# martinsbruveris/tensorflow-image-models

Measured on AMD Instinct MI355X. Metric: images/sec (fwd, bf16), higher is better.
Workload: dtype bf16; 1 GPU; resnet50 @224 fwd; per_gpu_batch=256, global_batch=256, parallelism=dp1, exchange=none, ranks=1, launcher=in-process, launch=hipGraph replay, 2 parallel branches of 128 images, branches=2

## Files before the change

### tensorflow-image-models_amd/csrc/gemm_chain_kernel.h

```cpp
#pragma once
#include "gemm_stream_kernel.h"

namespace tfimm_gemm {

struct ChainArgs {
  const bf16_t* x;
  const bf16_t* w1;
  const float* b1;
  const bf16_t* w2;
  const float* b2;
  const bf16_t* residual;
  const bf16_t* ds_x;
  const uint4* ds_w;
  bf16_t* out;
  int M, N2;
  int B, H, W;
  int ldw1, ldw2, ldr, ldc;
  int act1, act2;
  unsigned x_bytes, w1_bytes, w2_bytes, out_bytes, res_bytes, ds_bytes;
  int n_tiles;
  int dbg;
};

typedef void (*gemm_chain_fn)(const ChainArgs);

struct ChainGeom {
  static constexpr int BM = 128, NW = 4, C1 = 64, BN2 = 64;
  static constexpr int STRIP_ROWS = 256;
  static constexpr int STRIP_BYTES = STRIP_ROWS * 128;
  static constexpr int STAGE = 64 * 128;
#ifndef TFIMM_CHAIN_NST
#define TFIMM_CHAIN_NST 2
#endif
#ifndef TFIMM_CHAIN_WTN
#define TFIMM_CHAIN_WTN 64
#endif
  static constexpr int NST = TFIMM_CHAIN_NST;
  static constexpr int WTN = TFIMM_CHAIN_WTN;
  static constexpr int EPI_WAVE = 32 * WTN * 4;
  static constexpr int LDS_BYTES = STRIP_BYTES + NST * STAGE + NW * EPI_WAVE;
  static_assert(LDS_BYTES <= 80 * 1024, "two workgroups must fit one CU's 160 KiB of LDS");
};

template <int N>
__device__ __forceinline__ void chain_wait_vm() {
  asm volatile("s_waitcnt vmcnt(%0)" ::"n"(N) : "memory");
}

template <int I>
struct ChainIdx {
  static constexpr int value = I;
};

template <int NS2, int ACT = -1, bool DS = false>
__global__ void __launch_bounds__(256, 2) gemm_chain_kernel(const ChainArgs p) {
  using G = ChainGeom;
  constexpr int BM = G::BM, NW = G::NW, STAGE = G::STAGE, BN2 = G::BN2, NST = G::NST;
  constexpr int TN1 = 2;
  constexpr int STRIP_INSTR = G::STRIP_ROWS / 8 / NW;
  constexpr int B1_INSTR = 64 / 8 / NW;
  constexpr int B2_INSTR = BN2 / 8 / NW;
  constexpr int KS2 = 4;
  constexpr int TN2 = BN2 / 32;
  constexpr int NK1 = 9;
  typedef __attribute__((ext_vector_type(4))) unsigned int u32x4;

  extern __shared__ __attribute__((aligned(16))) char smem[];
  char* const sRing = smem + G::STRIP_BYTES;
  float* const sEpi = reinterpret_cast<float*>(smem + G::STRIP_BYTES + NST * STAGE);

  const int tid = threadIdx.x;
  const int lane = tid & 63;
  const int wave = __builtin_amdgcn_readfirstlane(tid >> 6);
  const int frow = lane & 31, fhi = lane >> 5;

  int t_first, t_hi, t_step;
  {
    const int nb = gridDim.x, bid = blockIdx.x;
    const int xcd = bid & 7, j = bid >> 3;
    const int q = p.n_tiles >> 3, r = p.n_tiles & 7;
    const int t_lo = xcd * q + (xcd < r ? xcd : r);
    t_hi = t_lo + q + (xcd < r ? 1 : 0);
    t_step = nb >> 3;
    t_first = t_lo + j;
  }
  if (t_first >= t_hi) return;

  const __amdgpu_buffer_rsrc_t rsrc_x = make_rsrc(p.x, p.x_bytes);
  const __amdgpu_buffer_rsrc_t rsrc_w1 = make_rsrc(p.w1, p.w1_bytes);
  const __amdgpu_buffer_rsrc_t rsrc_w2 = make_rsrc(p.w2, p.w2_bytes);
  const __amdgpu_buffer_rsrc_t rsrc_o = make_rsrc(p.out, p.out_bytes);
  const __amdgpu_buffer_rsrc_t rsrc_r = DS ? make_rsrc(p.ds_x, p.ds_bytes) : make_rsrc(p.residual, p.res_bytes);

  static_assert(NS2 >= 2, "the counted waits below are derived for at least two GEMM-2 steps");
  constexpr int LOOK = NST - 1;
  const int lrow = lane >> 3, lpc = lane & 7;

  unsigned b1_off[B1_INSTR], b2_off[B2_INSTR];
  int strip_chunk[STRIP_INSTR];
#pragma unroll
  for (int j = 0; j < B1_INSTR; ++j) {
    const int r = (wave * B1_INSTR + j) * 8 + lrow;
    b1_off[j] = (unsigned)(((size_t)r * p.ldw1 + (lpc ^ ((r >> 1) & 7)) * 8) * 2);
  }
#pragma unroll
  for (int j = 0; j < B2_INSTR; ++j) {
    const int r = (wave * B2_INSTR + j) * 8 + lrow;
    b2_off[j] = (unsigned)(((size_t)r * p.ldw2 + (lpc ^ ((r >> 1) & 7)) * 8) * 2);
  }
#pragma unroll
  for (int j = 0; j < STRIP_INSTR; ++j) {
    const int r = (wave * STRIP_INSTR + j) * 8 + lrow;
    strip_chunk[j] = (lpc ^ ((r >> 1) & 7)) * 16;
  }
  const int halo = p.W + 1;
  const int n_pix = p.B * p.H * p.W;
  auto issue_strip = [&](int tile, bool valid) __attribute__((always_inline)) {
    const int s0 = tile * BM - halo;
#pragma unroll
    for (int j = 0; j < STRIP_INSTR; ++j) {
      const int r = (wave * STRIP_INSTR + j) * 8 + lrow;
      const int s = s0 + r;
      const bool ok = valid && s >= 0 && s < n_pix;
      const unsigned off = ok ? (unsigned)s * 128u + (unsigned)strip_chunk[j] : kOobOffset;
      __builtin_amdgcn_raw_ptr_buffer_load_lds(rsrc_x, (lds_ptr_t)(smem + (wave * STRIP_INSTR + j) * 1024), 16, (int)off, 0, 0, 0);
    }
  };
  int iss_stage = 0;
  auto issue_step = [&](auto sc, int tile) __attribute__((always_inline)) {
    constexpr int S = decltype(sc)::value;
    constexpr int SL = S >= NK1 + NS2 ? S - NK1 - NS2 : S;
    const bool valid = S >= NK1 + NS2 ? (tile + t_step < t_hi) : true;
    char* const sa = sRing + iss_stage * STAGE;
    if constexpr (SL < NK1) {
#pragma unroll
      for (int j = 0; j < B1_INSTR; ++j) {
        const unsigned off = valid ? b1_off[j] : kOobOffset;
        __builtin_amdgcn_raw_ptr_buffer_load_lds(rsrc_w1, (lds_ptr_t)(sa + (wave * B1_INSTR + j) * 1024), 16, (int)off, SL * 128, 0, 0);
      }
    } else {
      const int soff = (int)((size_t)(SL - NK1) * BN2 * p.ldw2 * 2);
#pragma unroll
      for (int j = 0; j < B2_INSTR; ++j)
        __builtin_amdgcn_raw_ptr_buffer_load_lds(rsrc_w2, (lds_ptr_t)(sa + (wave * B2_INSTR + j) * 1024), 16, (int)b2_off[j], soff, 0, 0);
    }
    iss_stage = iss_stage == NST - 1 ? 0 : iss_stage + 1;
  };

  constexpr int WTN = G::WTN, LPR = WTN / 8, RPI = 64 / LPR, ITS = 32 / RPI;
  constexpr int PASSES = BN2 / WTN;
  constexpr int BPP = WTN / 32;
  constexpr int STORES = PASSES * ITS;
  constexpr int DS_X = DS ? 4 : 0;
  constexpr int DS_W = DS ? 8 : 0;
  constexpr int EPI_LOADS = (DS ? 0 : PASSES * ITS) + PASSES * 2;
  auto epi_slot = [](int row, int slot) -> int { return WTN == 64 ? (slot ^ (row & 15)) : (slot ^ ((row >> 1) & 7)); };
  const ActParams act1p = make_act(ACT >= 0 ? ACT : p.act1), act2p = make_act(ACT >= 0 ? ACT : p.act2);
  const int e_row = lane / LPR, e_c8 = lane % LPR;
  const bool has_res = !DS && p.residual != nullptr;
  float* const sEw = sEpi + wave * (G::EPI_WAVE / 4);

  struct Ops {
    static constexpr int all(int r) {
      if (DS && r == NK1 - 2) return B1_INSTR + TN1 * 4;
      if (r < NK1 - 1) return B1_INSTR;
      if (r == NK1 - 1) return EPI_LOADS + DS_X + B1_INSTR;
      const int u = r - NK1;
      return (u < NS2 - 1 ? EPI_LOADS : 0) + DS_W + B2_INSTR + (u == 0 ? STRIP_INSTR : 0) + STORES;
    }
    static constexpr int behind_dma(int r) {
      if (r < NK1) return 0;
      return (r - NK1 == 0 ? STRIP_INSTR : 0) + STORES;
    }
    static constexpr int wait_for(int r) {
      constexpr int T = NK1 + NS2;
      int n = behind_dma((r + T - LOOK) % T);
      for (int i = 1; i < LOOK; ++i) n += all((r + T - i) % T);
      return n;
    }
  };
  static_assert(B1_INSTR == B2_INSTR, "every weight step is two pieces per wave");
  static_assert(Ops::wait_for(NK1 + NS2 - 1) < 64, "vmcnt is a 6-bit counter");

  f32x4 bias1[TN1][4];
  auto load_bias1 = [&]() __attribute__((always_inline)) {
#pragma unroll
    for (int j = 0; j < TN1; ++j)
#pragma unroll
      for (int q = 0; q < 4; ++q) {
        const float4 b4 = *reinterpret_cast<const float4*>(p.b1 + j * 32 + q * 8 + fhi * 4);
        bias1[j][q] = f32x4{b4.x, b4.y, b4.z, b4.w};
      }
  };
  if constexpr (!DS) {
    load_bias1();
    asm volatile("s_waitcnt vmcnt(0)" : "+v"(bias1[0][0]), "+v"(bias1[0][3]), "+v"(bias1[TN1 - 1][0]), "+v"(bias1[TN1 - 1][3])::"memory");
  }

  if (TFIMM_PROBE(p.dbg) & 8) {
    const int n = ((blockIdx.x >> 3) & 7) * (TFIMM_PROBE(p.dbg) >> 8);
    for (int i = 0; i < n; ++i) asm volatile("s_sleep 8");
  }
  issue_strip(t_first, true);
  issue_step(ChainIdx<0>{}, t_first);
  if constexpr (LOOK > 1) issue_step(ChainIdx<1>{}, t_first);
  if constexpr (LOOK > 2) issue_step(ChainIdx<2>{}, t_first);
  static_assert(LOOK >= 1 && LOOK <= 3, "prologue written for up to three steps of lookahead");
  int cur = 0;
  bool first = true;
  auto rotate = [&]() __attribute__((always_inline)) { cur = cur == NST - 1 ? 0 : cur + 1; };

  for (int tile = t_first; tile < t_hi; tile += t_step) {
    const int m0 = tile * BM;

    unsigned vmask;
    {
      const int m = m0 + wave * 32 + frow;
      const int hw = p.H * p.W;
      const int rem = m % hw;
      const int oy = rem / p.W, ox = rem - oy * p.W;
      const unsigned vy = (oy > 0 ? 1u : 0u) | 2u | (oy + 1 < p.H ? 4u : 0u);
      const unsigned vx = (ox > 0 ? 1u : 0u) | 2u | (ox + 1 < p.W ? 4u : 0u);
      vmask = 0;
#pragma unroll
      for (int ky = 0; ky < 3; ++ky)
        if ((vy >> ky) & 1) vmask |= vx << (3 * ky);
      if (m >= p.M) vmask = 0;
    }

    f32x16 acc1[TN1];
#pragma unroll
    for (int j = 0; j < TN1; ++j)
#pragma unroll
      for (int e = 0; e < 16; ++e) acc1[j][e] = 0.f;
    uint4 rres[2][PASSES][ITS];
    u32x4 dsx[4];
    float4 braw[2][PASSES][2];
    const int e_m = m0 + wave * 32 + e_row;
    const int em = e_m < p.M ? e_m : p.M;
    const unsigned ldc2 = (unsigned)p.ldc * 2u, ldr2 = (unsigned)p.ldr * 2u;
    auto load_epi = [&](auto uc) __attribute__((always_inline)) {
      constexpr int u = decltype(uc)::value;
      const unsigned res_off0 = (unsigned)(((size_t)em * p.ldr + u * BN2 + e_c8 * 8) * 2);
#pragma unroll
      for (int g = 0; g < PASSES; ++g) {
        if constexpr (!DS) {
#pragma unroll
        for (int it = 0; it < ITS; ++it) {
          const unsigned off = res_off0 + (unsigned)(it * RPI) * ldr2 + (unsigned)(g * WTN * 2);
          rres[u & 1][g][it] = __builtin_bit_cast(uint4, __builtin_amdgcn_raw_buffer_load_b128(rsrc_r, (int)((TFIMM_PROBE(p.dbg) & 4) ? kOobOffset : off), 0, 0));
        }
        }
        braw[u & 1][g][0] = *reinterpret_cast<const float4*>(p.b2 + u * BN2 + g * WTN + e_c8 * 8);
        braw[u & 1][g][1] = *reinterpret_cast<const float4*>(p.b2 + u * BN2 + g * WTN + e_c8 * 8 + 4);
      }
    };
    auto tap_step = [&](auto kc) __attribute__((always_inline)) {
      constexpr int k = decltype(kc)::value;
      if constexpr (k < LOOK) { if (first) chain_wait_vm<(LOOK - 1) * B1_INSTR>(); else chain_wait_vm<Ops::wait_for(k)>(); }
      else chain_wait_vm<Ops::wait_for(k)>();
      tfimm_lds_reuse_barrier();
      if constexpr (DS && k == NK1 - 2) { load_bias1(); __builtin_amdgcn_sched_barrier(0); }
      if constexpr (k == NK1 - 1) {
        load_epi(ChainIdx<0>{});
        if constexpr (DS) {
          const unsigned xo = (unsigned)(m0 + wave * 32 + frow) * 128u + (unsigned)fhi * 16u;
#pragma unroll
          for (int t = 0; t < 4; ++t) dsx[t] = __builtin_amdgcn_raw_buffer_load_b128(rsrc_r, (int)(xo + t * 32), 0, 0);
        }
        __builtin_amdgcn_sched_barrier(0);
      }
      issue_step(ChainIdx<k + LOOK>{}, tile);
      if constexpr (k == NK1 - 1) __builtin_amdgcn_sched_barrier(0);
      constexpr int ky = k / 3, kx = k % 3;
      const bool ok = (vmask >> k) & 1;
      const uint4* sB = reinterpret_cast<const uint4*>(sRing + cur * STAGE);
      const int arow = wave * 32 + frow + ky * p.W + kx;
      u32x4 ua[4];
      {
        unsigned ra[4];
#pragma unroll
        for (int ks = 0; ks < 4; ++ks) ra[ks] = (unsigned)(size_t)(lds_ptr_t)(smem + lds_slot(arow, ks * 2 + fhi) * 16);
        asm volatile("ds_read_b128 %0, %4\n\tds_read_b128 %1, %5\n\tds_read_b128 %2, %6\n\tds_read_b128 %3, %7\n\t"
                     "s_waitcnt lgkmcnt(0)"
                     : "=&v"(ua[0]), "=&v"(ua[1]), "=&v"(ua[2]), "=&v"(ua[3])
                     : "v"(ra[0]), "v"(ra[1]), "v"(ra[2]), "v"(ra[3]) : "memory");
      }
#pragma unroll
      for (int ks = 0; ks < 4; ++ks) {
        const uint4 um = sel4(ok, __builtin_bit_cast(uint4, ua[ks]));
        const bf16x8 fa = __builtin_bit_cast(bf16x8, um);
        bf16x8 fb[TN1];
#pragma unroll
        for (int j = 0; j < TN1; ++j) fb[j] = __builtin_bit_cast(bf16x8, sB[lds_slot(j * 32 + frow, ks * 2 + fhi)]);
#pragma unroll
        for (int j = 0; j < TN1; ++j)
          if (!(TFIMM_PROBE(p.dbg) & 2)) acc1[j] = __builtin_amdgcn_mfma_f32_32x32x16_bf16(fb[j], fa, acc1[j], 0, 0, 0);
      }
      rotate();
    };
    tap_step(ChainIdx<0>{}); tap_step(ChainIdx<1>{}); tap_step(ChainIdx<2>{}); tap_step(ChainIdx<3>{}); tap_step(ChainIdx<4>{});
    tap_step(ChainIdx<5>{}); tap_step(ChainIdx<6>{}); tap_step(ChainIdx<7>{}); tap_step(ChainIdx<8>{});
    bf16x8 bmid[KS2];
#pragma unroll
    for (int j = 0; j < TN1; ++j)
#pragma unroll
      for (int q2 = 0; q2 < 2; ++q2) {
        tfimm_f32x2 v[4];
#pragma unroll
        for (int h2 = 0; h2 < 2; ++h2) {
          const int q = q2 * 2 + h2;
          const f32x4 b4 = bias1[j][q];
          v[h2 * 2 + 0] = tfimm_f32x2{acc1[j][q * 4 + 0] + b4[0], acc1[j][q * 4 + 1] + b4[1]};
          v[h2 * 2 + 1] = tfimm_f32x2{acc1[j][q * 4 + 2] + b4[2], acc1[j][q * 4 + 3] + b4[3]};
        }
        act8p(v, act1p);
        bmid[j * 2 + q2] = __builtin_bit_cast(bf16x8, pack8p(v));
      }

    auto slice_step = [&](auto uc) __attribute__((always_inline)) {
      constexpr int u = decltype(uc)::value;
      constexpr int n0 = u * BN2;
      const unsigned out_off0 = (unsigned)(((size_t)em * p.ldc + n0 + e_c8 * 8) * 2);
      chain_wait_vm<Ops::wait_for(NK1 + u)>();
      tfimm_lds_reuse_barrier();
      if constexpr (u + 1 < NS2) load_epi(ChainIdx<u + 1>{});
      u32x4 wds[TN2][4];
      if constexpr (DS) {
#pragma unroll
        for (int j = 0; j < TN2; ++j)
#pragma unroll
          for (int t = 0; t < 4; ++t) wds[j][t] = __builtin_bit_cast(u32x4, p.ds_w[(size_t)((u * TN2 + j) * 4 + t) * 64 + lane]);
      }
      __builtin_amdgcn_sched_barrier(0);
      issue_step(ChainIdx<NK1 + u + LOOK>{}, tile);
      if constexpr (u == 0) issue_strip(tile + t_step, tile + t_step < t_hi);
      __builtin_amdgcn_sched_barrier(0);

      f32x16 acc[TN2];
#pragma unroll
      for (int j = 0; j < TN2; ++j)
#pragma unroll
        for (int e = 0; e < 16; ++e) acc[j][e] = 0.f;
      {
        const uint4* sW = reinterpret_cast<const uint4*>(sRing + cur * STAGE);
#pragma unroll
        for (int t = 0; t < KS2; ++t) {
          bf16x8 fw[TN2];
#pragma unroll
          for (int j = 0; j < TN2; ++j) fw[j] = __builtin_bit_cast(bf16x8, sW[lds_slot(j * 32 + frow, t * 2 + fhi)]);
#pragma unroll
          for (int j = 0; j < TN2; ++j) acc[j] = __builtin_amdgcn_mfma_f32_32x32x16_bf16(fw[j], bmid[t], acc[j], 0, 0, 0);
        }
      }
      if constexpr (DS) {
#pragma unroll
        for (int t = 0; t < 4; ++t)
#pragma unroll
          for (int j = 0; j < TN2; ++j)
            acc[j] = __builtin_amdgcn_mfma_f32_32x32x16_bf16(__builtin_bit_cast(bf16x8, wds[j][t]), __builtin_bit_cast(bf16x8, dsx[t]),
                                                             acc[j], 0, 0, 0);
      }
      rotate();

      const bool skip_epi = (TFIMM_PROBE(p.dbg) & 1) != 0;
#pragma unroll
      for (int g = 0; g < PASSES; ++g) {
        asm volatile("s_nop 15\n\ts_nop 3" : "+v"(acc[g * BPP]), "+v"(acc[g * BPP + BPP - 1]));
#pragma unroll
        for (int j = 0; j < BPP; ++j)
#pragma unroll
          for (int q = 0; q < 4; ++q) {
            const int slot = j * 8 + q * 2 + fhi;
            const f32x16& a16 = acc[g * BPP + j];
            const f32x4 v = {a16[q * 4 + 0], a16[q * 4 + 1], a16[q * 4 + 2], a16[q * 4 + 3]};
            const unsigned addr = (unsigned)(size_t)(lds_ptr_t)(&sEw[frow * WTN + epi_slot(frow, slot) * 4]);
            asm volatile("ds_write_b128 %0, %1" ::"v"(addr), "v"(v) : "memory");
          }
        const float4 bq0 = braw[u & 1][g][0], bq1 = braw[u & 1][g][1];
        const tfimm_f32x2 bias2[4] = {{bq0.x, bq0.y}, {bq0.z, bq0.w}, {bq1.x, bq1.y}, {bq1.z, bq1.w}};
#pragma unroll
        for (int ip = 0; ip < ITS; ip += 2) {
        f32x4 st[4];
        {
          unsigned ra[4];
#pragma unroll
          for (int w = 0; w < 2; ++w) {
            const int pr = (ip + w) * RPI + e_row;
            ra[2 * w] = (unsigned)(size_t)(lds_ptr_t)(&sEw[pr * WTN + epi_slot(pr, 2 * e_c8) * 4]);
            ra[2 * w + 1] = (unsigned)(size_t)(lds_ptr_t)(&sEw[pr * WTN + epi_slot(pr, 2 * e_c8 + 1) * 4]);
          }
          asm volatile("ds_read_b128 %0, %4\n\tds_read_b128 %1, %5\n\tds_read_b128 %2, %6\n\tds_read_b128 %3, %7\n\t"
                       "s_waitcnt lgkmcnt(0)"
                       : "=&v"(st[0]), "=&v"(st[1]), "=&v"(st[2]), "=&v"(st[3])
                       : "v"(ra[0]), "v"(ra[1]), "v"(ra[2]), "v"(ra[3]) : "memory");
        }
#pragma unroll
        for (int w = 0; w < 2; ++w) {
          const int it = ip + w;
          const f32x4 lo = st[2 * w], hi = st[2 * w + 1];
          tfimm_f32x2 v[4] = {{lo[0], lo[1]}, {lo[2], lo[3]}, {hi[0], hi[1]}, {hi[2], hi[3]}};
#pragma unroll
          for (int e = 0; e < 4; ++e) v[e] += bias2[e];
          if (has_res) {
            asm volatile("");
            tfimm_f32x2 r2[4];
            unpack8p(rres[u & 1][g][it], r2);
#pragma unroll
            for (int e = 0; e < 4; ++e) v[e] += r2[e];
          }
          act8p(v, act2p);
          const unsigned off = out_off0 + (unsigned)(it * RPI) * ldc2 + (unsigned)(g * WTN * 2);
          __builtin_amdgcn_raw_buffer_store_b128(__builtin_bit_cast(u32x4, pack8p(v)), rsrc_o,
                                                 (int)(skip_epi ? kOobOffset : off), 0, 0);
        }
        }
      }
    };
    slice_step(ChainIdx<0>{});
    slice_step(ChainIdx<1>{});
    if constexpr (NS2 > 2) slice_step(ChainIdx<2>{});
    if constexpr (NS2 > 3) slice_step(ChainIdx<3>{});
    if constexpr (NS2 > 4) { slice_step(ChainIdx<4>{}); slice_step(ChainIdx<5>{}); slice_step(ChainIdx<6>{}); slice_step(ChainIdx<7>{}); }
    static_assert(NS2 == 2 || NS2 == 3 || NS2 == 4 || NS2 == 8, "instantiate the slice steps of this NS2");
    first = false;
  }
  asm volatile("s_waitcnt vmcnt(0)" ::: "memory");
}

}
```

Before: 75760 images/sec.

## Stream downsample weights through the LDS ring as extra pipeline steps

In the downsample variant of the fused chain kernel, the per-slice downsample weights used to be loaded straight from global memory into registers just before the MFMAs. They now arrive by buffer-to-LDS DMA as an extra step in the weight ring, so each GEMM-2 slice has two steps, and the vmcnt wait bookkeeping is updated to match. The bias-1 load is also moved up front for all variants, which drops its mid-loop load. The aim is to hide the global-load latency and register pressure of the downsample weights, at the cost of more pipeline steps, barriers and LDS ring turnover.

```diff
diff --git a/tensorflow-image-models_amd/csrc/gemm_chain_kernel.h b/tensorflow-image-models_amd/csrc/gemm_chain_kernel.h
--- a/tensorflow-image-models_amd/csrc/gemm_chain_kernel.h
+++ b/tensorflow-image-models_amd/csrc/gemm_chain_kernel.h
@@ -91,9 +91,12 @@
   const __amdgpu_buffer_rsrc_t rsrc_w2 = make_rsrc(p.w2, p.w2_bytes);
   const __amdgpu_buffer_rsrc_t rsrc_o = make_rsrc(p.out, p.out_bytes);
   const __amdgpu_buffer_rsrc_t rsrc_r = DS ? make_rsrc(p.ds_x, p.ds_bytes) : make_rsrc(p.residual, p.res_bytes);
+  const __amdgpu_buffer_rsrc_t rsrc_d = make_rsrc(p.ds_w, DS ? (unsigned)p.N2 * 128u : 0u);
 
   static_assert(NS2 >= 2, "the counted waits below are derived for at least two GEMM-2 steps");
   constexpr int LOOK = NST - 1;
+  constexpr int SPS = DS ? 2 : 1;
+  constexpr int T = NK1 + SPS * NS2;
   const int lrow = lane >> 3, lpc = lane & 7;
 
   unsigned b1_off[B1_INSTR], b2_off[B2_INSTR];
@@ -129,8 +132,9 @@
   int iss_stage = 0;
   auto issue_step = [&](auto sc, int tile) __attribute__((always_inline)) {
     constexpr int S = decltype(sc)::value;
-    constexpr int SL = S >= NK1 + NS2 ? S - NK1 - NS2 : S;
-    const bool valid = S >= NK1 + NS2 ? (tile + t_step < t_hi) : true;
+    constexpr int SL = S >= T ? S - T : S;
+    static_assert(SL < T, "a step looks ahead into the next tile's program at most");
+    const bool valid = S >= T ? (tile + t_step < t_hi) : true;
     char* const sa = sRing + iss_stage * STAGE;
     if constexpr (SL < NK1) {
 #pragma unroll
@@ -138,8 +142,15 @@
         const unsigned off = valid ? b1_off[j] : kOobOffset;
         __builtin_amdgcn_raw_ptr_buffer_load_lds(rsrc_w1, (lds_ptr_t)(sa + (wave * B1_INSTR + j) * 1024), 16, (int)off, SL * 128, 0, 0);
       }
+    } else if constexpr (DS && ((SL - NK1) & 1)) {
+      constexpr int soff = ((SL - NK1) >> 1) * STAGE;
+#pragma unroll
+      for (int j = 0; j < B2_INSTR; ++j) {
+        const unsigned off = (TFIMM_PROBE(p.dbg) & 16) ? kOobOffset : (unsigned)((wave * B2_INSTR + j) * 1024 + lane * 16);
+        __builtin_amdgcn_raw_ptr_buffer_load_lds(rsrc_d, (lds_ptr_t)(sa + (wave * B2_INSTR + j) * 1024), 16, (int)off, soff, 0, 0);
+      }
     } else {
-      const int soff = (int)((size_t)(SL - NK1) * BN2 * p.ldw2 * 2);
+      const int soff = (int)((size_t)((SL - NK1) / SPS) * BN2 * p.ldw2 * 2);
 #pragma unroll
       for (int j = 0; j < B2_INSTR; ++j)
         __builtin_amdgcn_raw_ptr_buffer_load_lds(rsrc_w2, (lds_ptr_t)(sa + (wave * B2_INSTR + j) * 1024), 16, (int)b2_off[j], soff, 0, 0);
@@ -152,7 +163,6 @@
   constexpr int BPP = WTN / 32;
   constexpr int STORES = PASSES * ITS;
   constexpr int DS_X = DS ? 4 : 0;
-  constexpr int DS_W = DS ? 8 : 0;
   constexpr int EPI_LOADS = (DS ? 0 : PASSES * ITS) + PASSES * 2;
   auto epi_slot = [](int row, int slot) -> int { return WTN == 64 ? (slot ^ (row & 15)) : (slot ^ ((row >> 1) & 7)); };
   const ActParams act1p = make_act(ACT >= 0 ? ACT : p.act1), act2p = make_act(ACT >= 0 ? ACT : p.act2);
@@ -162,40 +172,36 @@
 
   struct Ops {
     static constexpr int all(int r) {
-      if (DS && r == NK1 - 2) return B1_INSTR + TN1 * 4;
       if (r < NK1 - 1) return B1_INSTR;
       if (r == NK1 - 1) return EPI_LOADS + DS_X + B1_INSTR;
-      const int u = r - NK1;
-      return (u < NS2 - 1 ? EPI_LOADS : 0) + DS_W + B2_INSTR + (u == 0 ? STRIP_INSTR : 0) + STORES;
+      const int u = (r - NK1) / SPS;
+      const bool w2 = !DS || ((r - NK1) & 1) == 0, last = !DS || ((r - NK1) & 1) == 1;
+      return (w2 && u < NS2 - 1 ? EPI_LOADS : 0) + B2_INSTR + (w2 && u == 0 ? STRIP_INSTR : 0) + (last ? STORES : 0);
     }
     static constexpr int behind_dma(int r) {
       if (r < NK1) return 0;
-      return (r - NK1 == 0 ? STRIP_INSTR : 0) + STORES;
+      const int u = (r - NK1) / SPS;
+      const bool w2 = !DS || ((r - NK1) & 1) == 0, last = !DS || ((r - NK1) & 1) == 1;
+      return (w2 && u == 0 ? STRIP_INSTR : 0) + (last ? STORES : 0);
     }
     static constexpr int wait_for(int r) {
-      constexpr int T = NK1 + NS2;
       int n = behind_dma((r + T - LOOK) % T);
       for (int i = 1; i < LOOK; ++i) n += all((r + T - i) % T);
       return n;
     }
   };
   static_assert(B1_INSTR == B2_INSTR, "every weight step is two pieces per wave");
-  static_assert(Ops::wait_for(NK1 + NS2 - 1) < 64, "vmcnt is a 6-bit counter");
+  static_assert(Ops::wait_for(T - 1) < 64 && Ops::wait_for(NK1 + 1) < 64, "vmcnt is a 6-bit counter");
 
   f32x4 bias1[TN1][4];
-  auto load_bias1 = [&]() __attribute__((always_inline)) {
-#pragma unroll
-    for (int j = 0; j < TN1; ++j)
-#pragma unroll
-      for (int q = 0; q < 4; ++q) {
-        const float4 b4 = *reinterpret_cast<const float4*>(p.b1 + j * 32 + q * 8 + fhi * 4);
-        bias1[j][q] = f32x4{b4.x, b4.y, b4.z, b4.w};
-      }
-  };
-  if constexpr (!DS) {
-    load_bias1();
-    asm volatile("s_waitcnt vmcnt(0)" : "+v"(bias1[0][0]), "+v"(bias1[0][3]), "+v"(bias1[TN1 - 1][0]), "+v"(bias1[TN1 - 1][3])::"memory");
-  }
+#pragma unroll
+  for (int j = 0; j < TN1; ++j)
+#pragma unroll
+    for (int q = 0; q < 4; ++q) {
+      const float4 b4 = *reinterpret_cast<const float4*>(p.b1 + j * 32 + q * 8 + fhi * 4);
+      bias1[j][q] = f32x4{b4.x, b4.y, b4.z, b4.w};
+    }
+  asm volatile("s_waitcnt vmcnt(0)" : "+v"(bias1[0][0]), "+v"(bias1[0][3]), "+v"(bias1[TN1 - 1][0]), "+v"(bias1[TN1 - 1][3])::"memory");
 
   if (TFIMM_PROBE(p.dbg) & 8) {
     const int n = ((blockIdx.x >> 3) & 7) * (TFIMM_PROBE(p.dbg) >> 8);
@@ -260,7 +266,6 @@
       if constexpr (k < LOOK) { if (first) chain_wait_vm<(LOOK - 1) * B1_INSTR>(); else chain_wait_vm<Ops::wait_for(k)>(); }
       else chain_wait_vm<Ops::wait_for(k)>();
       tfimm_lds_reuse_barrier();
-      if constexpr (DS && k == NK1 - 2) { load_bias1(); __builtin_amdgcn_sched_barrier(0); }
       if constexpr (k == NK1 - 1) {
         load_epi(ChainIdx<0>{});
         if constexpr (DS) {
@@ -321,19 +326,13 @@
     auto slice_step = [&](auto uc) __attribute__((always_inline)) {
       constexpr int u = decltype(uc)::value;
       constexpr int n0 = u * BN2;
+      constexpr int R = NK1 + SPS * u;
       const unsigned out_off0 = (unsigned)(((size_t)em * p.ldc + n0 + e_c8 * 8) * 2);
-      chain_wait_vm<Ops::wait_for(NK1 + u)>();
+      chain_wait_vm<Ops::wait_for(R)>();
       tfimm_lds_reuse_barrier();
       if constexpr (u + 1 < NS2) load_epi(ChainIdx<u + 1>{});
-      u32x4 wds[TN2][4];
-      if constexpr (DS) {
-#pragma unroll
-        for (int j = 0; j < TN2; ++j)
-#pragma unroll
-          for (int t = 0; t < 4; ++t) wds[j][t] = __builtin_bit_cast(u32x4, p.ds_w[(size_t)((u * TN2 + j) * 4 + t) * 64 + lane]);
-      }
       __builtin_amdgcn_sched_barrier(0);
-      issue_step(ChainIdx<NK1 + u + LOOK>{}, tile);
+      issue_step(ChainIdx<R + LOOK>{}, tile);
       if constexpr (u == 0) issue_strip(tile + t_step, tile + t_step < t_hi);
       __builtin_amdgcn_sched_barrier(0);
 
@@ -354,12 +353,22 @@
         }
       }
       if constexpr (DS) {
-#pragma unroll
-        for (int t = 0; t < 4; ++t)
+        rotate();
+        chain_wait_vm<Ops::wait_for(R + 1)>();
+        tfimm_lds_reuse_barrier();
+        __builtin_amdgcn_sched_barrier(0);
+        issue_step(ChainIdx<R + 1 + LOOK>{}, tile);
+        __builtin_amdgcn_sched_barrier(0);
+        const uint4* sD = reinterpret_cast<const uint4*>(sRing + cur * STAGE);
+#pragma unroll
+        for (int t = 0; t < 4; ++t) {
+          bf16x8 fd[TN2];
+#pragma unroll
+          for (int j = 0; j < TN2; ++j) fd[j] = __builtin_bit_cast(bf16x8, sD[(j * 4 + t) * 64 + lane]);
 #pragma unroll
           for (int j = 0; j < TN2; ++j)
-            acc[j] = __builtin_amdgcn_mfma_f32_32x32x16_bf16(__builtin_bit_cast(bf16x8, wds[j][t]), __builtin_bit_cast(bf16x8, dsx[t]),
-                                                             acc[j], 0, 0, 0);
+            acc[j] = __builtin_amdgcn_mfma_f32_32x32x16_bf16(fd[j], __builtin_bit_cast(bf16x8, dsx[t]), acc[j], 0, 0, 0);
+        }
       }
       rotate();
 
```

Result: slower. 74570 images/sec (-1.6%).
